# radiocosmology/cora

Measured on AMD Instinct MI355X. Metric: sky-maps/sec (nside=1024, lmax=2048, 256 freq), higher is better.
Workload: dtype f64

## Files before the change

### cora_amd/csrc/clarray.hip

```cpp
#include "common.h"

#include <cstring>
#include <type_traits>

#define CL_MAXZ 17

#define CL_XS 512
#define CL_LPT 9

__global__ void cl_transpose_kernel(const double *__restrict__ dd, const double *__restrict__ dv,
                                    const double *__restrict__ vv, int nkperp, int nkpar, double *__restrict__ tt) {
    __shared__ double tile[32][33];
    const double *src = blockIdx.z == 0 ? dd : (blockIdx.z == 1 ? dv : vv);
    double *dst = tt + (size_t)blockIdx.z * nkpar * CL_XS;
    const int x0 = blockIdx.y * 32, y0 = blockIdx.x * 32;
    const int tx = threadIdx.x & 31, ty = threadIdx.x >> 5;
    for (int r = ty; r < 32; r += 8) {
        const int x = x0 + r, y = y0 + tx;
        tile[r][tx] = (x < nkperp && y < nkpar) ? src[(size_t)x * nkpar + y] : 0.0;
    }
    __syncthreads();
    for (int r = ty; r < 32; r += 8) {
        const int y = y0 + r, x = x0 + tx;
        if (y < nkpar && x < CL_XS) dst[(size_t)y * CL_XS + x] = (x < nkperp) ? tile[tx][r] : 0.0;
    }
}

template <int ZINT>
__global__ void __launch_bounds__(256)
clarray21_kernel(const double *__restrict__ tt, int nkperp, int nkpar, double kperpmin, double xscale, double yscale,
                 const double *__restrict__ chi, const double *__restrict__ pfd, const double *__restrict__ fz,
                 const double *__restrict__ bz, int F, int zint_rt, const double *__restrict__ w,
                 const double *__restrict__ log10l, int nl, int l_base, const int2 *__restrict__ pairs,
                 double *__restrict__ scratch, int nl_total, int l_block) {
    const int zint = ZINT > 0 ? ZINT : zint_rt;
    extern __shared__ __attribute__((aligned(16))) double sm[];
    double *prof = sm;
    double *lxcs_s = sm + zint * (CL_XS + 2);
    double *par = lxcs_s + zint;
    int *ipar = reinterpret_cast<int *>(par + zint * zint * 8);
    const int PS = CL_XS + 2;
    const int tid = threadIdx.x;
    const int i = pairs[blockIdx.x].x, j = pairs[blockIdx.x].y;
    if (i < 0) return;
    const double ux = (double)nkperp - 1e-5, uy = (double)nkpar - 1e-5;
    const size_t tsz = (size_t)nkpar * CL_XS;

    double lxs[CL_LPT], acc[CL_LPT];
#pragma unroll
    for (int k = 0; k < CL_LPT; k++) {
        const int li = l_base + tid + 256 * k;
        lxs[k] = log10l[min(li, nl_total - 1)] * xscale;
        acc[k] = 0.0;
    }
    const int l_end = min(nl_total, l_base + 256 * CL_LPT);
    const double lx_lo = log10l[l_base] * xscale, lx_hi = log10l[l_end - 1] * xscale;
    const int kmax = (l_end - l_base + 255) / 256;

    int noclamp = 1;
    for (int t = tid; t < zint * zint; t += 256) {
        const int a = t / zint, b = t - a * zint;
        const int za = i * zint + a, zb = j * zint + b;
        const double x1 = chi[za], x2 = chi[zb];
        const double xc = 0.5 * (x1 + x2);
        const double lxc = log10(xc * kperpmin) * xscale;
        double yy = fabs(x2 - x1) * yscale;
        yy = yy < 0.0 ? 0.0 : (yy > uy ? uy : yy);
        int y0 = (int)yy;
        double wy = yy - (double)y0;
        if (y0 + 1 > nkpar - 1) {
            y0 = nkpar - 2;
            wy = 1.0;
        }
        const double W = w[a] * w[b] * pfd[za] * pfd[zb] / (xc * xc * M_PI);
        const double cdd = W * bz[za] * bz[zb];
        const double cdv = W * (fz[za] * bz[zb] + fz[zb] * bz[za]);
        const double cvv = W * fz[za] * fz[zb];
        double *pp = par + t * 8;
        pp[0] = cdd * (1.0 - wy);
        pp[1] = cdd * wy;
        pp[2] = cdv * (1.0 - wy);
        pp[3] = cdv * wy;
        pp[4] = cvv * (1.0 - wy);
        pp[5] = cvv * wy;
        pp[6] = lxc;
        double xhi = lx_hi - lxc, xlo = lx_lo - lxc;
        xhi = xhi < 0.0 ? 0.0 : (xhi > ux ? ux : xhi);
        xlo = xlo < 0.0 ? 0.0 : (xlo > ux ? ux : xlo);
        ipar[t * 4 + 0] = y0;
        ipar[t * 4 + 1] = (int)xlo;
        ipar[t * 4 + 2] = min((int)xhi + 2, nkperp);
        const double x2nd = (l_base + 1 < l_end ? log10l[l_base + 1] * xscale : lx_hi) - lxc;
        if (!(x2nd >= 0.0 && lx_hi - lxc <= ux)) noclamp = 0;
    }
    const bool all_fast = __syncthreads_and(noclamp) != 0;
    __shared__ int s_nsp;
    __shared__ double s_lxk[32];
    if (tid < 32) s_lxk[tid] = log10l[min(l_base + tid, nl_total - 1)] * xscale;
    if (tid < 64) {
        bool wide = false;
        if (l_base + tid + 1 < l_end) wide = (log10l[l_base + tid + 1] - log10l[l_base + tid]) * xscale >= 2.0;
        const unsigned long long m = __ballot(wide);
        if (tid == 0) s_nsp = m == ~0ull ? 32 : min(32, (int)__builtin_ctzll(~m));
    }

    for (int a = 0; a < zint; a++) {
        __syncthreads();
        if (ZINT > 0 && all_fast) {
            constexpr int ZN = ZINT > 0 ? ZINT : 1;
            const int nsp = min(s_nsp, l_end - l_base);
            const double lxd = log10l[min(l_base + nsp, nl_total - 1)] * xscale;
            int xlo = nkperp, xhi = 0;
#pragma unroll
            for (int b = 0; b < ZN; b++) {
                const double xx = fmin(fmax(lxd - par[(a * ZN + b) * 8 + 6], 0.0), ux);
                xlo = min(xlo, (int)xx);
                xhi = max(xhi, ipar[(a * ZN + b) * 4 + 2]);
            }
            if (nsp >= l_end - l_base) xlo = xhi;
            auto combine = [&](int b, const double (&v)[6]) {
                const double *pp = par + (a * ZN + b) * 8;
                return pp[0] * v[0] + pp[1] * v[1] + pp[2] * v[2] + pp[3] * v[3] + pp[4] * v[4] + pp[5] * v[5];
            };
            {
                constexpr int ZH = (ZN + 1) / 2;
                const int hb = tid >> 7, b0 = hb ? ZH : 0, nb = hb ? ZN - ZH : ZH;
                constexpr int QB = 3;
                for (int x = (xlo & ~1) + 2 * (tid & 127); x < xhi; x += 256) {
#pragma unroll
                    for (int q0 = 0; q0 < ZH; q0 += QB) {
                        double2 v[QB][6];
#pragma unroll
                        for (int q = 0; q < QB; q++) {
                            if (q0 + q < nb) {
                                const double *r0 = tt + (size_t)ipar[(a * ZN + b0 + q0 + q) * 4 + 0] * CL_XS + x, *r1 = r0 + CL_XS;
                                v[q][0] = *reinterpret_cast<const double2 *>(r0);
                                v[q][1] = *reinterpret_cast<const double2 *>(r1);
                                v[q][2] = *reinterpret_cast<const double2 *>(r0 + tsz);
                                v[q][3] = *reinterpret_cast<const double2 *>(r1 + tsz);
                                v[q][4] = *reinterpret_cast<const double2 *>(r0 + 2 * tsz);
                                v[q][5] = *reinterpret_cast<const double2 *>(r1 + 2 * tsz);
                            }
                        }
#pragma unroll
                        for (int q = 0; q < QB; q++) {
                            if (q0 + q < nb) {
                                const double *pp = par + (a * ZN + b0 + q0 + q) * 8;
                                double2 o;
                                o.x = pp[0] * v[q][0].x + pp[1] * v[q][1].x + pp[2] * v[q][2].x + pp[3] * v[q][3].x + pp[4] * v[q][4].x + pp[5] * v[q][5].x;
                                o.y = pp[0] * v[q][0].y + pp[1] * v[q][1].y + pp[2] * v[q][2].y + pp[3] * v[q][3].y + pp[4] * v[q][4].y + pp[5] * v[q][5].y;
                                *reinterpret_cast<double2 *>(prof + (b0 + q0 + q) * PS + x) = o;
                            }
// ... 20 lines not shown
            if (xhi == nkperp) {
                __syncthreads();
                if (tid < ZN) prof[tid * PS + nkperp] = prof[tid * PS + nkperp - 1];
            }
        } else
        for (int b = 0; b < zint; b++) {
            const int t = a * zint + b;
            const double *pp = par + t * 8;
            const double c0 = pp[0], c1 = pp[1], c2 = pp[2], c3 = pp[3], c4 = pp[4], c5 = pp[5];
            const int y0 = ipar[t * 4 + 0], x0r = ipar[t * 4 + 1], nx = ipar[t * 4 + 2];
            const double *r0 = tt + (size_t)y0 * CL_XS, *r1 = r0 + CL_XS;
            double *pb = prof + b * PS;
            for (int x = x0r + tid; x < nx; x += 256)
                pb[x] = c0 * r0[x] + c1 * r1[x] + c2 * r0[tsz + x] + c3 * r1[tsz + x] + c4 * r0[2 * tsz + x] +
                        c5 * r1[2 * tsz + x];
            if (tid == 0) lxcs_s[b] = pp[6];
            if (nx == nkperp && tid == ((nkperp - 1 - x0r) & 255)) pb[nkperp] = pb[nkperp - 1];
        }
        __syncthreads();
        double lxc_r[ZINT > 0 ? ZINT : 1];
        if constexpr (ZINT > 0) {
#pragma unroll
            for (int b = 0; b < ZINT; b++) lxc_r[b] = lxcs_s[b];
        }
        auto interp = [&](int b, double lx, double lxc, bool clamp) {
            double xx = lx - lxc;
            if (clamp) xx = fmin(fmax(xx, 0.0), ux);
            const int x0 = (int)xx;
            const double wx = __builtin_amdgcn_fract(xx);
            const double *pr = prof + b * PS + x0;
            const double s0 = pr[0], s1 = pr[1];
            return fma(wx, s1 - s0, s0);
        };
        auto interp_all = [&](auto fast_c) {
            constexpr bool FAST = decltype(fast_c)::value;
#pragma unroll
            for (int k = 0; k < CL_LPT; k++) {
                if (k < kmax && (k < kmax - 1 || l_base + tid + 256 * k < nl_total)) {
                    const bool clamp = !FAST || (k == 0 && tid == 0);
                    double s = 0.0;
                    if constexpr (ZINT > 0) {
#pragma unroll
                        for (int b = 0; b < ZINT; b++) s += interp(b, lxs[k], lxc_r[b], clamp);
                    } else {
                        for (int b = 0; b < zint; b++) s += interp(b, lxs[k], lxcs_s[b], clamp);
                    }
                    acc[k] += s;
                }
            }
        };
        if (all_fast) interp_all(std::true_type{});
        else interp_all(std::false_type{});
    }
#pragma unroll
    for (int k = 0; k < CL_LPT; k++) {
        const int li = l_base + tid + 256 * k;
        if (li < nl_total)
            scratch[((size_t)(li / l_block) * gridDim.x + blockIdx.x) * l_block + li % l_block] = acc[k];
    }
}

#define CL_BAND 32
__host__ __device__ static inline long cl_band_count(int n) {
    return n >= CL_BAND ? (long)CL_BAND * (n - (CL_BAND - 1)) + (long)(CL_BAND - 1) * CL_BAND / 2 : (long)n * (n + 1) / 2;
}
__host__ __device__ static inline int2 pair_of_index(long p, int F) {
    int B = 0;
    for (;; B++) {
        const long c = cl_band_count(F - CL_BAND * B);
        if (p < c) break;
        p -= c;
    }
    const int n = F - CL_BAND * B;
    const int nfull = n >= CL_BAND ? n - (CL_BAND - 1) : 0;
    int i, dd;
    if (p < (long)nfull * CL_BAND) {
        const int xq = (int)(p & 7), sq = (int)(p >> 3);
        i = sq >> 2;
        dd = 4 * xq + (sq & 3);
    } else {
        p -= (long)nfull * CL_BAND;
        int e = n >= CL_BAND ? CL_BAND - 1 : n;
        i = nfull;
        while (p >= e) {
            p -= e;
            e--;
// ... 127 lines not shown
                           const double *log10l, int nl, int pair_first, int pair_step, long npl_pad, int l_block,
                           double *out_pairs) {
    const size_t tt_bytes = sizeof(double) * 3 * (size_t)nkpar * CL_XS;
    double *tt = nullptr;
    int2 *dpairs = nullptr;
    int rc;
    if ((rc = corahip_ctx_scratch(ctx, 0, tt_bytes, (void **)&tt))) return rc;
    if ((rc = corahip_ctx_scratch(ctx, 2, sizeof(int2) * npl_pad, (void **)&dpairs))) return rc;
    const long key[4] = {F, pair_first, pair_step, npl_pad};
    if (ctx->pairs_ptr != (void *)dpairs || memcmp(key, ctx->pairs_key, sizeof(key)) != 0) {
        std::vector<int2> pairs((size_t)npl_pad, make_int2(-1, -1));
        long p = 0, k = 0;
        const long npairs_all = (long)F * (F + 1) / 2;
        for (; p < npairs_all; p++)
            if (p >= pair_first && (p - pair_first) % pair_step == 0) pairs[(size_t)k++] = pair_of_index(p, F);
        HIP_TRY(hipMemcpyAsync(dpairs, pairs.data(), sizeof(int2) * npl_pad, hipMemcpyHostToDevice, ctx->stream));
        HIP_TRY(hipStreamSynchronize(ctx->stream));
        memcpy(ctx->pairs_key, key, sizeof(key));
        ctx->pairs_ptr = (void *)dpairs;
    }
    const bool pinned = ctx->tt_pinned && ctx->tt_pin[0] == dd && ctx->tt_pin[1] == dv && ctx->tt_pin[2] == vv;
    if (!(pinned && ctx->tt_valid && ctx->tt_stream == ctx->stream && ctx->scratch_bytes[0] == tt_bytes)) {
        dim3 grid((nkpar + 31) / 32, CL_XS / 32, 3);
        cl_transpose_kernel<<<grid, 256, 0, ctx->stream>>>(dd, dv, vv, nkperp, nkpar, tt);
        LAUNCH_CHECK();
        ctx->tt_valid = pinned;
        ctx->tt_stream = ctx->stream;
    }
    const double xscale = (double)(nkperp - 1) / log10(kperpmax / kperpmin);
    const double yscale = kparmax / M_PI;
    const size_t shm = sizeof(double) * ((size_t)zint * (CL_XS + 2) + zint + (size_t)zint * zint * 10);
    auto kern = zint == 9 ? clarray21_kernel<9> : (zint == 5 ? clarray21_kernel<5> : (zint == 3 ? clarray21_kernel<3> : clarray21_kernel<0>));
    HIP_TRY(hipFuncSetAttribute((const void *)kern, hipFuncAttributeMaxDynamicSharedMemorySize, (int)shm));
    for (int l_base = 0; l_base < nl; l_base += 256 * CL_LPT) {
        kern<<<(unsigned)npl_pad, 256, shm, ctx->stream>>>(tt, nkperp, nkpar, kperpmin, xscale, yscale, chi, pfd, f, b, F, zint, w,
                                                          log10l, nl, l_base, dpairs, out_pairs, nl, l_block);
        LAUNCH_CHECK();
    }
    return 0;
}

int corahip_clarray_tables_pin(corahip_ctx *ctx, const double *dd, const double *dv, const double *vv, uint64_t generation) {
    ARG_CHECK(ctx != nullptr);
    if (dd == nullptr && generation != 0 && !(ctx->tt_pinned && ctx->tt_pin_gen == generation))
        return 0;
    const bool same = ctx->tt_pinned && dd && ctx->tt_pin[0] == dd && ctx->tt_pin[1] == dv && ctx->tt_pin[2] == vv &&
                      ctx->tt_pin_gen == generation;
    if (same) return 0;
    ctx->tt_pin[0] = dd;
    ctx->tt_pin[1] = dv;
    ctx->tt_pin[2] = vv;
    ctx->tt_pin_gen = generation;
    ctx->tt_pinned = dd != nullptr;
    ctx->tt_valid = false;
    return 0;
}

int corahip_clarray_table21cm(corahip_ctx *ctx, const double *dd, const double *dv, const double *vv, int nkperp,
                              int nkpar, double kperpmin, double kperpmax, double kparmax, const double *chi,
                              const double *pfd, const double *f, const double *b, int F, int zint, const double *w,
                              const double *log10l, int nl, double *out) {
    ARG_CHECK(ctx != nullptr && dd && dv && vv && chi && pfd && f && b && w && log10l && out);
    ARG_CHECK(nkperp >= 2 && nkperp < CL_XS && nkpar >= 2 && F >= 1 && zint >= 1 && zint <= CL_MAXZ && nl >= 1);
    ARG_CHECK(kperpmin > 0 && kperpmax > kperpmin && kparmax > 0);
    StageTimer t(ctx, "clarray");
    const long npairs = (long)F * (F + 1) / 2;
    double *scratch = nullptr;
    int rc;
    if ((rc = corahip_ctx_scratch(ctx, 1, sizeof(double) * (size_t)npairs * nl, (void **)&scratch))) return rc;
// ... 73 lines not shown
```

### cora_amd/csrc/common.h

```cpp
#pragma once
#include <hip/hip_runtime.h>

#include <cstdarg>
#include <cstdint>
#include <cstdio>
#include <map>
#include <string>
#include <type_traits>
#include <vector>

#include "../../include/corahip.h"
#include "dev_buf.h"

void corahip_set_error(const char *fmt, ...);

struct corahip_prof_entry {
    double total_ms = 0.0;
    int launches = 0;
};

struct corahip_pending_event {
    std::string name;
    hipEvent_t e0, e1;
};

struct corahip_linefft_plan {
    int n = 0, P = 0, logP = 0, blu = 0;
    int Pct = 0;
    dev_buf<double2> filt_ct;
    dev_buf<double2> tw;
    dev_buf<double2> chirp;
    dev_buf<double2> filt;
    dev_buf<double2> rtw;
};

#define CORAHIP_NSCRATCH 13
struct corahip_ctx {
    int device = 0;
    hipStream_t stream = nullptr;
    hipStream_t stream2 = nullptr;
    hipEvent_t ev_fork = nullptr, ev_join = nullptr;
    dev_buf<int> k5_tickets;
    dev_buf<unsigned> draw_slot_tab;
    int draw_slot_lmax = -1;
    bool mt_plist_ready = false;
    hipStream_t gen_stream = nullptr;
    hipEvent_t ev_ring[8] = {};
    const void *draw_pending = nullptr;
    hipEvent_t t0 = nullptr, t1 = nullptr;
    bool profile = false;
    std::map<std::string, corahip_prof_entry> prof;
    std::vector<corahip_pending_event> pending;
    int num_cu = 256;
    size_t total_mem = 0;
    dev_buf<char> scratch[CORAHIP_NSCRATCH];
    size_t scratch_bytes[CORAHIP_NSCRATCH] = {};
    int debug_poison = -1;
    const void *tt_pin[3] = {nullptr, nullptr, nullptr};
    uint64_t tt_pin_gen = 0;
    bool tt_pinned = false, tt_valid = false;
    hipStream_t tt_stream = nullptr;
    long pairs_key[4] = {-1, -1, -1, -1};
    void *pairs_ptr = nullptr;
    std::map<int, corahip_linefft_plan> linefft;
};

int corahip_ctx_scratch(corahip_ctx *ctx, int slot, size_t bytes, void **out);
int corahip_debug_fill(corahip_ctx *ctx, void *p, size_t bytes);

struct StageTimer {
    corahip_ctx *ctx;
    hipEvent_t e0 = nullptr, e1 = nullptr;
    const char *name;
    hipStream_t stream;
    StageTimer(corahip_ctx *c, const char *n, hipStream_t on = nullptr, bool other = false) : ctx(c), name(n), stream(other ? on : c->stream) {
        if (ctx->profile) {
            (void)hipEventCreate(&e0);
// ... 113 lines not shown
```

### cora_amd/csrc/draw.hip

```cpp
#include "common.h"

#include <cstdlib>
#include <type_traits>

#include "rng_dev.h"
#include "stream_internal.h"

__device__ static inline double2 philox_normal_pair(uint64_t seed, int l, int F, int nup, int m,
                                                    const double2 *lg = RNG_LOG_TAB, const double2 *sc = RNG_SC_TAB) {
    const uint64_t ctr = ((uint64_t)((uint32_t)l * (uint32_t)F + (uint32_t)nup) << 32) | (uint32_t)m;
    return philox_boxmuller(ctr, seed, lg, sc);
}

__global__ void normals_kernel(uint64_t seed, int lmax, int F, double *__restrict__ g) {
    const int l = blockIdx.y;
    const int lp1 = l + 1;
    const long n = (long)F * lp1;
    double *gl = g + (size_t)F * l * lp1;
    for (long q = (long)blockIdx.x * blockDim.x + threadIdx.x; q < n; q += (long)gridDim.x * blockDim.x) {
        const int m = (int)(q % lp1);
        const int nup = (int)(q / lp1);
        const double2 v = philox_normal_pair(seed, l, F, nup, m);
        gl[q] = v.x;
        gl[n + q] = v.y;
// ... 68 lines not shown
            }
        }
    }

    const double sc = 0.70710678118654752440;
    const long base = alm_idx(l, 0, lmax);
#pragma unroll
    for (int t = 0; t < NCT; t++) {
        const int col = col0 + 16 * t + ri;
        if (col >= 4 * Gout) continue;
#pragma unroll
        for (int r = 0; r < 4; r++) {
            const int ro = row0 + wave * 16 + kq + 4 * r;
            if (ro < nrow) {
                const int c = ro >= lp1 ? 1 : 0;
                const int m = ro - c * lp1;
                const long idx = (long)m * (2 * lmax + 1 - m) / 2 + l;
                (void)base;
                alm[((size_t)idx * Gout + (col >> 2)) * 8 + c * 4 + (col & 3)] = acc[t][r] * sc;
            }
        }
    }
}

__device__ static inline void draw_glds16(const void *gsrc, unsigned lds_byte_addr) {
    unsigned keep;
    const unsigned dst = __builtin_amdgcn_readfirstlane(lds_byte_addr);
    asm volatile("s_mov_b32 %0, m0\n\ts_mov_b32 m0, %2\n\ts_nop 0\n\tglobal_load_lds_dwordx4 %1, off\n\ts_mov_b32 m0, %0"
                 : "=&s"(keep)
                 : "v"(gsrc), "s"(dst)
                 : "memory");
}

#ifndef DRAW_STAMPS
#define DRAW_STAMPS 0
#endif
#if DRAW_STAMPS
__device__ unsigned long long g_draw_stamps[8];
#define DSTAMP(k) { unsigned long long _t; asm volatile("s_memtime %0\n\ts_waitcnt lgkmcnt(0)" : "=s"(_t)::"memory"); d_acc[k] += _t - d_last; d_last = _t; }
#else
#define DSTAMP(k)
#endif

#define DRAW_WAVES 8
#define DRAW_MB (16 * DRAW_WAVES)
#define DRAW_NBUF 3

static inline long draw_slots(int l_lo, int l_hi) {
    long n = 0;
    for (int l = l_lo; l <= l_hi; l++) n += (l / DRAW_MB) + 1;
    return n;
}

template <int NCT, bool FROMG = false, int NB = DRAW_NBUF>
__global__ void __launch_bounds__(64 * DRAW_WAVES, 2)
draw_rng_kernel(const double *__restrict__ T, size_t t_ldl, int rows, const int32_t *__restrict__ info,
                const double *__restrict__ zeros, uint64_t seed, const double *__restrict__ gsrc, size_t g_off, int l_lo,
                int l_hi, int lmax, int F, int nu0, int nu1, int cw, int nnu, int Gout, int nslots, int ncg0, int ncg,
                double *__restrict__ alm, unsigned *__restrict__ queue, const unsigned *__restrict__ slot_tab) {
    constexpr int NC = 16 * NCT;
    constexpr int ROWD = DRAW_KC;
    constexpr int BUF = NC * ROWD;
    constexpr int QPW = (NC / 4 + DRAW_WAVES - 1) / DRAW_WAVES;
    static_assert(QPW * DRAW_WAVES == NC / 4 || NC / 4 < DRAW_WAVES, "every staging wave issues the same number of pieces");
    extern __shared__ __attribute__((aligned(16))) double lds[];
    static_assert(NB == 3, "the counted waits below assume three stages");
    __shared__ double2 lg_s[257], sc_s[256];
    __shared__ int s_next[2];

    const int tid = threadIdx.x, lane = tid & 63;
    const int wave = __builtin_amdgcn_readfirstlane(tid >> 6);
    const int ri = lane & 15, kq = lane >> 4;
    const int nitems = nslots * ncg;
    const unsigned lds_base = (unsigned)(size_t)(__attribute__((address_space(3))) double *)lds;
#if DRAW_STAMPS
    unsigned long long d_acc[8] = {0, 0, 0, 0, 0, 0, 0, 0}, d_last;
    { unsigned long long _t; asm volatile("s_memtime %0\n\ts_waitcnt lgkmcnt(0)" : "=s"(_t)::"memory"); d_last = _t; }
#endif

    struct item_t {
        int l, mb, base0, lbase, lend, kmax, nchunk, c_full;
        bool tri_tail;
        const double *Tl;
// ... 190 lines not shown
                return __hiloint2double(hi, lo);
            };
#pragma unroll
            for (int t = 0; t < NCT; t++) {
                const int col = cur_lbase + 16 * t + (ri & ~3);
                const bool col_ok = col < cur_lend4;
#pragma unroll
                for (int r = 0; r < 4; r++) {
                    const double re = acc0[t][r] * sc, im = acc1[t][r] * sc;
                    const double re_a = quad(re, std::integral_constant<int, 0x88>{});
                    const double im_a = quad(im, std::integral_constant<int, 0x88>{});
                    const double re_b = quad(re, std::integral_constant<int, 0xDD>{});
                    const double im_b = quad(im, std::integral_constant<int, 0xDD>{});
                    const int m = mw + kq + 4 * r;
                    if (col_ok && m < lp1) {
                        const long idx = (long)m * (2 * lmax + 1 - m) / 2 + l;
                        *reinterpret_cast<double2 *>(alm + ((size_t)idx * Gout + (col >> 2)) * 8 + 2 * q) =
                            upper ? make_double2(im_a, im_b) : make_double2(re_a, re_b);
                    }
                }
            }
        }
        DSTAMP(5);
        if (!have_next) break;
    }
#if DRAW_STAMPS
    if (lane == 0) {
        for (int k = 0; k < 7; k++) atomicAdd(&g_draw_stamps[k], d_acc[k]);
        atomicAdd(&g_draw_stamps[7], 1ull);
    }
#endif
}

struct draw_chan {
    int nu0, nu1, cw, nnu;
};
static int draw_slot_table(corahip_ctx *ctx, int lmax, const unsigned **tab) {
    if (ctx->draw_slot_tab && ctx->draw_slot_lmax == lmax) {
        *tab = ctx->draw_slot_tab;
        return 0;
    }
    std::vector<unsigned> h;
    h.reserve((size_t)draw_slots(0, lmax));
    for (int l = lmax; l >= 0; l--)
        for (int mb = 0; mb <= l / DRAW_MB; mb++) h.push_back(((unsigned)l << 8) | (unsigned)mb);
    (void)ctx->draw_slot_tab.reset();
    ctx->draw_slot_lmax = -1;
    dev_buf<unsigned> d;
    HIP_TRY(d.alloc(h.size()));
    HIP_TRY(hipMemcpy(d, h.data(), sizeof(unsigned) * h.size(), hipMemcpyHostToDevice));
    ctx->draw_slot_tab = std::move(d);
    ctx->draw_slot_lmax = lmax;
    *tab = ctx->draw_slot_tab;
    return 0;
}

template <int NCT, bool FROMG = false, int NB = DRAW_NBUF>
static int launch_draw_rng(corahip_ctx *ctx, hipStream_t stream, const double *T, size_t t_ldl, int rows, const int32_t *info,
                           uint64_t seed, const double *gsrc, size_t g_off, int l_lo, int l_hi, int lmax, int F,
                           draw_chan ch, int Gout, double *alm) {
    constexpr int NC = 16 * NCT;
    const size_t shm = sizeof(double) * NB * NC * DRAW_KC;
    HIP_TRY(hipFuncSetAttribute((const void *)draw_rng_kernel<NCT, FROMG, NB>, hipFuncAttributeMaxDynamicSharedMemorySize,
                                (int)shm));
    char *zq = nullptr;
    int rc = corahip_ctx_scratch(ctx, 3, 8192, (void **)&zq);
    if (rc) return rc;
    HIP_TRY(hipMemsetAsync(zq, 0, 8192, stream));
    const int n0 = std::min(ch.cw, ch.nnu), n1 = ch.nnu - n0;
    const int ncg0 = (((n0 + 3) & ~3) + NC - 1) / NC, ncg = ncg0 + (((n1 + 3) & ~3) + NC - 1) / NC;
    const long nslots = draw_slots(l_lo, l_hi);
    const long nitems = nslots * ncg;
    ARG_CHECK(nitems < (1L << 30) && lmax < (1 << 24) && lmax / DRAW_MB < 256);
    const unsigned *slot_tab = nullptr;
    if ((rc = draw_slot_table(ctx, lmax, &slot_tab))) return rc;
    slot_tab += l_hi < lmax ? draw_slots(l_hi + 1, lmax) : 0;
    const int per_cu = (shm + 8300 > 80 * 1024) ? 1 : 2;
    dim3 grid((unsigned)std::min<long>(nitems, (long)ctx->num_cu * per_cu));
    draw_rng_kernel<NCT, FROMG, NB><<<grid, 64 * DRAW_WAVES, shm, stream>>>(T, t_ldl, rows, info, (const double *)zq, seed, gsrc,
                                                                        g_off, l_lo, l_hi, lmax, F, ch.nu0, ch.nu1, ch.cw,
                                                                        ch.nnu, Gout, (int)nslots, ncg0, ncg, alm,
                                                                        (unsigned *)(zq + 4096), slot_tab);
    LAUNCH_CHECK();
#if DRAW_STAMPS
    {
        unsigned long long hs[8], z[8] = {0};
        HIP_TRY(hipStreamSynchronize(stream));
        HIP_TRY(hipMemcpyFromSymbol(hs, HIP_SYMBOL(g_draw_stamps), sizeof(hs)));
        const double per = 1.0 / (double)std::max<unsigned long long>(hs[7], 1);
        fprintf(stderr, "K3 NCT=%d waves=%llu: cycles/wave  prologue %.0f wait+barrier %.0f (first chunk of an item %.0f) stage-issue %.0f rng+mfma %.0f next-item %.0f epilogue %.0f\n",
                NCT, hs[7], hs[0] * per, hs[1] * per, hs[6] * per, hs[2] * per, hs[3] * per, hs[4] * per, hs[5] * per);
        HIP_TRY(hipMemcpyToSymbol(HIP_SYMBOL(g_draw_stamps), z, sizeof(z)));
    }
#endif
    return 0;
}

__global__ void dev_to_square_kernel(const double *__restrict__ alm, int lmax, int nnu, int G,
                                     double *__restrict__ sq) {
    const int L = lmax + 1;
    const long n = (long)nnu * L * L;
    for (long q = (long)blockIdx.x * blockDim.x + threadIdx.x; q < n; q += (long)gridDim.x * blockDim.x) {
        const int m = (int)(q % L);
        const int l = (int)((q / L) % L);
        const int nu = (int)(q / ((long)L * L));
        double2 v = make_double2(0.0, 0.0);
        if (m <= l) {
            const long idx = (long)m * (2 * lmax + 1 - m) / 2 + l;
            const double *cell = alm + ((size_t)idx * G + (nu >> 2)) * 8 + (nu & 3);
            v = make_double2(cell[0], cell[4]);
        }
        *reinterpret_cast<double2 *>(sq + 2 * q) = v;
    }
}

// ... 53 lines not shown
        if (ncol <= 16) return launch_draw_rng<1, true>(ctx, stream, T, t_ldl, rows, info, 0, g, g_off, l_lo, l_hi, lmax, F, ch, Gout, alm_dev);
        if (ncol <= 32) return launch_draw_rng<2, true>(ctx, stream, T, t_ldl, rows, info, 0, g, g_off, l_lo, l_hi, lmax, F, ch, Gout, alm_dev);
        if (ncol <= 64) return launch_draw_rng<4, true>(ctx, stream, T, t_ldl, rows, info, 0, g, g_off, l_lo, l_hi, lmax, F, ch, Gout, alm_dev);
        return launch_draw_rng<8, true>(ctx, stream, T, t_ldl, rows, info, 0, g, g_off, l_lo, l_hi, lmax, F, ch, Gout, alm_dev);
    }
    ARG_CHECK(!chan_folded(ch));
    const int ncol = 4 * Gout, nu0 = ch.nu0, nnu = ch.nnu, t_row0 = rows ? nu0 : 0;
    if (ncol <= 16) return launch_draw<1>(ctx, stream, T, t_ldl, t_row0, info, g, g_off, l_lo, l_hi, lmax, F, nu0, nnu, Gout, alm_dev);
    if (ncol <= 32) return launch_draw<2>(ctx, stream, T, t_ldl, t_row0, info, g, g_off, l_lo, l_hi, lmax, F, nu0, nnu, Gout, alm_dev);
    if (ncol <= 64) return launch_draw<4>(ctx, stream, T, t_ldl, t_row0, info, g, g_off, l_lo, l_hi, lmax, F, nu0, nnu, Gout, alm_dev);
    if (ncol <= 128) return launch_draw<8>(ctx, stream, T, t_ldl, t_row0, info, g, g_off, l_lo, l_hi, lmax, F, nu0, nnu, Gout, alm_dev);
    return launch_draw<16>(ctx, stream, T, t_ldl, t_row0, info, g, g_off, l_lo, l_hi, lmax, F, nu0, nnu, Gout, alm_dev);
}

static int draw_host_stream(corahip_ctx *ctx, const double *T, int rows, const int32_t *info, const double *g, int lmax, int F,
                            draw_chan ch, double *alm_dev) {
    StageTimer t(ctx, "draw");
    return draw_stream_range(ctx, ctx->stream, T, rows, info, g, 0, 0, lmax, lmax, F, ch, alm_dev);
}

static int draw_philox(corahip_ctx *ctx, const double *T, int rows, const int32_t *info, uint64_t seed, int lmax, int F,
                       draw_chan ch, double *alm_dev) {
    if (F & 1) {
        double *g = nullptr;
        int rc = corahip_ctx_scratch(ctx, 1, sizeof(double) * 2 * (size_t)F * nalm_of(lmax), (void **)&g);
        if (rc) return rc;
        if ((rc = corahip_normals_philox(ctx, seed, lmax, F, g))) return rc;
        return draw_host_stream(ctx, T, rows, info, g, lmax, F, ch, alm_dev);
    }
    StageTimer t(ctx, "draw");
    const int Gout = (ch.nnu + 3) / 4;
    const size_t t_ldl = rows ? (size_t)ch.nnu * F : (size_t)F * F;
    const int ncol = chan_ncol(ch);
    if (ncol <= 16) return launch_draw_rng<1>(ctx, ctx->stream, T, t_ldl, rows, info, seed, nullptr, 0, 0, lmax, lmax, F, ch, Gout, alm_dev);
    if (ncol <= 32) return launch_draw_rng<2>(ctx, ctx->stream, T, t_ldl, rows, info, seed, nullptr, 0, 0, lmax, lmax, F, ch, Gout, alm_dev);
    if (ncol <= 64) return launch_draw_rng<4>(ctx, ctx->stream, T, t_ldl, rows, info, seed, nullptr, 0, 0, lmax, lmax, F, ch, Gout, alm_dev);
    return launch_draw_rng<8>(ctx, ctx->stream, T, t_ldl, rows, info, seed, nullptr, 0, 0, lmax, lmax, F, ch, Gout, alm_dev);
}

static int chan_of(const corahip_chanset *set, int F, draw_chan &ch) {
    ARG_CHECK(set != nullptr && (set->nchunks == 1 || set->nchunks == 2) && set->chunk_nnu >= 1);
    ARG_CHECK(set->nu0[0] >= 0 && set->nu0[0] + set->chunk_nnu <= F);
    if (set->nchunks == 2) {
        ARG_CHECK(set->chunk_nnu % 4 == 0);
        ARG_CHECK(set->nu0[1] >= set->nu0[0] + set->chunk_nnu && set->nu0[1] + set->chunk_nnu <= F);
        ch = draw_chan{set->nu0[0], set->nu0[1], set->chunk_nnu, 2 * set->chunk_nnu};
    } else {
        ch = draw_chan{set->nu0[0], 0, set->chunk_nnu, set->chunk_nnu};
    }
    return 0;
}

int corahip_draw_alm_philox(corahip_ctx *ctx, const double *T, const int32_t *info, uint64_t seed, int lmax, int F,
                            int nu0, int nnu, double *alm_dev) {
    ARG_CHECK(ctx != nullptr && T != nullptr && alm_dev != nullptr);
    ARG_CHECK(lmax >= 0 && F >= 1 && nu0 >= 0 && nnu >= 1 && nu0 + nnu <= F);
    return draw_philox(ctx, T, 0, info, seed, lmax, F, draw_chan{nu0, 0, nnu, nnu}, alm_dev);
}

int corahip_draw_alm_philox_rows(corahip_ctx *ctx, const double *T_rows, const int32_t *info, uint64_t seed, int lmax,
                                 int F, int nu0, int nnu, double *alm_dev) {
    ARG_CHECK(ctx != nullptr && T_rows != nullptr && alm_dev != nullptr);
    ARG_CHECK(lmax >= 0 && F >= 1 && nu0 >= 0 && nnu >= 1 && nu0 + nnu <= F);
    return draw_philox(ctx, T_rows, 1, info, seed, lmax, F, draw_chan{nu0, 0, nnu, nnu}, alm_dev);
}

// ... 54 lines not shown
```

Measured before the change: 3298.

## Replace per-l sub-sample interpolation with knot-based row sums in clarray kernel

When all sub-sample centre offsets lie within half a cell of a central offset, the kernel accumulates per-column row sums S and first-moment sums E over the z sub-samples. Each l is then evaluated with one linear interpolation of S corrected by E, instead of interpolating every sub-sample separately. Multipoles whose bracketing cell is ambiguous are put on a dirty list and still go through the exact per-sample path. The change also adds a launch-bounds occupancy hint and extra shared memory, and is on by default with an environment variable to disable it.

```diff
diff --git a/cora_amd/csrc/clarray.hip b/cora_amd/csrc/clarray.hip
--- a/cora_amd/csrc/clarray.hip
+++ b/cora_amd/csrc/clarray.hip
@@ -7,6 +7,9 @@
 
 #define CL_XS 512
 #define CL_LPT 9
+#define CL_KN_CAP 512
+#define CL_KN_MARGIN 0x1p-20
+#define CL_KN_DMAX (0.5 - 0x1p-20)
 
 __global__ void cl_transpose_kernel(const double *__restrict__ dd, const double *__restrict__ dv,
                                     const double *__restrict__ vv, int nkperp, int nkpar, double *__restrict__ tt) {
@@ -26,13 +29,18 @@
     }
 }
 
+__device__ static inline double cl_mul_rn(double a, double b) {
+#pragma clang fp contract(off)
+    return a * b;
+}
+
 template <int ZINT>
-__global__ void __launch_bounds__(256)
+__global__ void __launch_bounds__(256, 3)
 clarray21_kernel(const double *__restrict__ tt, int nkperp, int nkpar, double kperpmin, double xscale, double yscale,
                  const double *__restrict__ chi, const double *__restrict__ pfd, const double *__restrict__ fz,
                  const double *__restrict__ bz, int F, int zint_rt, const double *__restrict__ w,
                  const double *__restrict__ log10l, int nl, int l_base, const int2 *__restrict__ pairs,
-                 double *__restrict__ scratch, int nl_total, int l_block) {
+                 double *__restrict__ scratch, int nl_total, int l_block, int knots_on) {
     const int zint = ZINT > 0 ? ZINT : zint_rt;
     extern __shared__ __attribute__((aligned(16))) double sm[];
     double *prof = sm;
@@ -96,7 +104,7 @@
     const bool all_fast = __syncthreads_and(noclamp) != 0;
     __shared__ int s_nsp;
     __shared__ double s_lxk[32];
-    if (tid < 32) s_lxk[tid] = log10l[min(l_base + tid, nl_total - 1)] * xscale;
+    if (tid < 32) s_lxk[tid] = cl_mul_rn(log10l[min(l_base + tid, nl_total - 1)], xscale);
     if (tid < 64) {
         bool wide = false;
         if (l_base + tid + 1 < l_end) wide = (log10l[l_base + tid + 1] - log10l[l_base + tid]) * xscale >= 2.0;
@@ -104,7 +112,86 @@
         if (tid == 0) s_nsp = m == ~0ull ? 32 : min(32, (int)__builtin_ctzll(~m));
     }
 
-    for (int a = 0; a < zint; a++) {
+    constexpr int ZQ = ZINT > 0 ? ZINT : 1;
+    __shared__ double s_dlim[2];
+    __shared__ int s_kok, s_ndirty;
+    __shared__ unsigned short s_dlist[CL_KN_CAP];
+    __shared__ double s_dlx[CL_KN_CAP];
+    __shared__ double s_early[32][4];
+    bool knots = false, kn_early = false, kn_eclean = false;
+    unsigned kn_dirty = 0;
+    double cstar = 0.0;
+    double kn_S[2] = {0.0, 0.0}, kn_E[2] = {0.0, 0.0};
+    double kn_lacc[CL_KN_CAP / 256];
+    int kn_lidx[CL_KN_CAP / 256];
+    int kn_xlo = 0, kn_xhi = 0;
+    if constexpr (ZINT > 0) {
+        if (knots_on && all_fast) {
+            if (tid < 64) {
+                const double c0 = par[((ZQ / 2) * ZQ + ZQ / 2) * 8 + 6];
+                double lo = 0.0, hi = 0.0;
+                int ok = 1;
+                for (int t = tid; t < ZQ * ZQ; t += 64) {
+                    const double d = par[t * 8 + 6] - c0;
+                    par[t * 8 + 7] = d;
+                    lo = fmin(lo, d);
+                    hi = fmax(hi, d);
+                    if (ipar[t * 4 + 2] == nkperp) ok = 0;
+                }
+#pragma unroll
+                for (int s = 32; s >= 1; s >>= 1) {
+                    lo = fmin(lo, __shfl_xor(lo, s));
+                    hi = fmax(hi, __shfl_xor(hi, s));
+                    ok &= __shfl_xor(ok, s);
+                }
+                if (tid == 0) {
+                    s_dlim[0] = lo;
+                    s_dlim[1] = hi;
+                    s_kok = ok && fmax(-lo, hi) < CL_KN_DMAX;
+                    s_ndirty = 0;
+                }
+            }
+            __syncthreads();
+            knots = s_kok != 0;
+        }
+        if (knots) {
+            cstar = par[((ZQ / 2) * ZQ + ZQ / 2) * 8 + 6];
+            const double dmin = s_dlim[0], dmax = s_dlim[1];
+            const int nsp = min(s_nsp, l_end - l_base);
+            kn_early = tid < nsp;
+            if (tid < 32) s_early[tid][0] = s_early[tid][1] = s_early[tid][2] = s_early[tid][3] = 0.0;
+#pragma unroll
+            for (int k = 0; k < CL_LPT; k++) {
+                const int e = tid + 256 * k;
+                if (l_base + e >= nl_total) continue;
+                const double lxe = cl_mul_rn(log10l[l_base + e], xscale);
+                const double xs = lxe - cstar;
+                const double lo = xs - dmax - CL_KN_MARGIN, hi = xs - dmin + CL_KN_MARGIN;
+                const bool clean = lo >= 0.0 && (int)lo == (int)hi;
+                if (k == 0 && kn_early) {
+                    kn_eclean = clean;
+                } else if (!clean) {
+                    kn_dirty |= 1u << k;
+                    const int slot = atomicAdd(&s_ndirty, 1);
+                    if (slot < CL_KN_CAP) {
+                        s_dlist[slot] = (unsigned short)e;
+                        s_dlx[slot] = lxe;
+                    }
+                }
+            }
+            __syncthreads();
+            const int nd = s_ndirty;
+            if (nd > CL_KN_CAP) knots = false;
+#pragma unroll
+            for (int q = 0; q < CL_KN_CAP / 256; q++) {
+                kn_lidx[q] = (knots && tid + 256 * q < nd) ? (int)s_dlist[tid + 256 * q] : -1;
+                kn_lacc[q] = 0.0;
+            }
+        }
+    }
+
+    auto round = [&](int a, auto kn_c) {
+        constexpr bool KN = decltype(kn_c)::value;
         __syncthreads();
         if (ZINT > 0 && all_fast) {
             constexpr int ZN = ZINT > 0 ? ZINT : 1;
@@ -118,6 +205,8 @@
                 xhi = max(xhi, ipar[(a * ZN + b) * 4 + 2]);
             }
             if (nsp >= l_end - l_base) xlo = xhi;
+            kn_xlo = xlo & ~1;
+            kn_xhi = xhi;
             auto combine = [&](int b, const double (&v)[6]) {
                 const double *pp = par + (a * ZN + b) * 8;
                 return pp[0] * v[0] + pp[1] * v[1] + pp[2] * v[2] + pp[3] * v[3] + pp[4] * v[4] + pp[5] * v[5];
@@ -204,6 +293,46 @@
             const double s0 = pr[0], s1 = pr[1];
             return fma(wx, s1 - s0, s0);
         };
+        if constexpr (ZINT > 0 && KN) {
+            const double *dl_r = par + a * ZQ * 8 + 7;
+            auto rowsum = [&](int x, double &S, double &E) {
+                const double *pr = prof + x;
+                double t = pr[0], e = dl_r[0] * t;
+#pragma unroll
+                for (int b = 1; b < ZQ; b++) {
+                    const double s = pr[b * PS];
+                    t += s;
+                    e = fma(dl_r[8 * b], s, e);
+                }
+                S += t;
+                E += e;
+            };
+            auto sub_sum = [&](double lx) {
+                double s = 0.0;
+#pragma unroll
+                for (int b = 0; b < ZQ; b++) s += interp(b, lx, lxc_r[b], true);
+                return s;
+            };
+#pragma unroll
+            for (int r = 0; r < 2; r++) {
+                const int x = tid + 256 * r;
+                if (x >= kn_xlo && x < kn_xhi) rowsum(x, kn_S[r], kn_E[r]);
+            }
+            if (kn_early) {
+                double *se = s_early[tid];
+                if (kn_eclean) {
+                    const int x = (int)(s_lxk[tid] - cstar);
+                    rowsum(x, se[0], se[2]);
+                    rowsum(x + 1, se[1], se[3]);
+                } else {
+                    se[0] += sub_sum(s_lxk[tid]);
+                }
+            }
+#pragma unroll
+            for (int q = 0; q < CL_KN_CAP / 256; q++)
+                if (kn_lidx[q] >= 0) kn_lacc[q] += sub_sum(s_dlx[tid + 256 * q]);
+            return;
+        }
         auto interp_all = [&](auto fast_c) {
             constexpr bool FAST = decltype(fast_c)::value;
 #pragma unroll
@@ -223,7 +352,47 @@
         };
         if (all_fast) interp_all(std::true_type{});
         else interp_all(std::false_type{});
-    }
+    };
+    auto slot_of = [&](int li) {
+        return ((size_t)(li / l_block) * gridDim.x + blockIdx.x) * l_block + li % l_block;
+    };
+    if constexpr (ZINT > 0) {
+        if (knots) {
+            for (int a = 0; a < ZINT; a++) round(a, std::true_type{});
+            __syncthreads();
+#pragma unroll
+            for (int r = 0; r < 2; r++) {
+                prof[tid + 256 * r] = kn_S[r];
+                prof[PS + tid + 256 * r] = kn_E[r];
+            }
+            __syncthreads();
+            auto knot_value = [](double xs, double S0, double S1, double E0, double E1) {
+                return fma(__builtin_amdgcn_fract(xs), S1 - S0, S0) - (E1 - E0);
+            };
+#pragma unroll
+            for (int k = 0; k < CL_LPT; k++) {
+                const int li = l_base + tid + 256 * k;
+                if (li >= nl_total) continue;
+                double v;
+                if (k == 0 && kn_early) {
+                    const double *se = s_early[tid];
+                    v = kn_eclean ? knot_value(s_lxk[tid] - cstar, se[0], se[1], se[2], se[3]) : se[0];
+                } else if ((kn_dirty >> k) & 1) {
+                    continue;
+                } else {
+                    const double xs = cl_mul_rn(log10l[li], xscale) - cstar;
+                    const double *pr = prof + (int)xs;
+                    v = knot_value(xs, pr[0], pr[1], pr[PS], pr[PS + 1]);
+                }
+                scratch[slot_of(li)] = v;
+            }
+#pragma unroll
+            for (int q = 0; q < CL_KN_CAP / 256; q++)
+                if (kn_lidx[q] >= 0) scratch[slot_of(l_base + kn_lidx[q])] = kn_lacc[q];
+            return;
+        }
+    }
+    for (int a = 0; a < zint; a++) round(a, std::false_type{});
 #pragma unroll
     for (int k = 0; k < CL_LPT; k++) {
         const int li = l_base + tid + 256 * k;
@@ -417,9 +586,11 @@
     const size_t shm = sizeof(double) * ((size_t)zint * (CL_XS + 2) + zint + (size_t)zint * zint * 10);
     auto kern = zint == 9 ? clarray21_kernel<9> : (zint == 5 ? clarray21_kernel<5> : (zint == 3 ? clarray21_kernel<3> : clarray21_kernel<0>));
     HIP_TRY(hipFuncSetAttribute((const void *)kern, hipFuncAttributeMaxDynamicSharedMemorySize, (int)shm));
+    const char *kn_env = getenv("CORAHIP_K1_KNOTS");
+    const int knots_on = !(kn_env && kn_env[0] == '0' && kn_env[1] == 0);
     for (int l_base = 0; l_base < nl; l_base += 256 * CL_LPT) {
         kern<<<(unsigned)npl_pad, 256, shm, ctx->stream>>>(tt, nkperp, nkpar, kperpmin, xscale, yscale, chi, pfd, f, b, F, zint, w,
-                                                          log10l, nl, l_base, dpairs, out_pairs, nl, l_block);
+                                                          log10l, nl, l_base, dpairs, out_pairs, nl, l_block, knots_on);
         LAUNCH_CHECK();
     }
     return 0;
```

Result: no change. 3325 (median of 6 runs) (+0.8%).

## Add wide 256-column draw kernel with half-height m blocks for large channel counts

Applied to the files above, without the earlier changes.

Adds a new draw kernel that covers 256 output columns per block, with 16 MFMA tiles per wave and only 8 m rows per wave. It uses double-buffered LDS staging fed by scalar-base global-to-LDS loads. For more than 128 channels, one block now handles all frequencies, so the Philox normals are generated once per (l,m) instead of once per column group. The slot table becomes per-m-block-size. The trade-off is higher accumulator register pressure, larger LDS use, and smaller m blocks that need more work items.

```diff
diff --git a/cora_amd/csrc/common.h b/cora_amd/csrc/common.h
--- a/cora_amd/csrc/common.h
+++ b/cora_amd/csrc/common.h
@@ -41,8 +41,8 @@
     hipStream_t stream2 = nullptr;
     hipEvent_t ev_fork = nullptr, ev_join = nullptr;
     dev_buf<int> k5_tickets;
-    dev_buf<unsigned> draw_slot_tab;
-    int draw_slot_lmax = -1;
+    dev_buf<unsigned> draw_slot_tab[2];
+    int draw_slot_lmax[2] = {-1, -1};
     bool mt_plist_ready = false;
     hipStream_t gen_stream = nullptr;
     hipEvent_t ev_ring[8] = {};
diff --git a/cora_amd/csrc/draw.hip b/cora_amd/csrc/draw.hip
--- a/cora_amd/csrc/draw.hip
+++ b/cora_amd/csrc/draw.hip
@@ -124,6 +124,15 @@
                  : "memory");
 }
 
+__device__ static inline void draw_glds16_s(const void *sbase, unsigned lane_byte_off, unsigned lds_byte_addr) {
+    unsigned keep;
+    const unsigned dst = __builtin_amdgcn_readfirstlane(lds_byte_addr);
+    asm volatile("s_mov_b32 %0, m0\n\ts_mov_b32 m0, %3\n\ts_nop 0\n\tglobal_load_lds_dwordx4 %1, %2\n\ts_mov_b32 m0, %0"
+                 : "=&s"(keep)
+                 : "v"(lane_byte_off), "s"(sbase), "s"(dst)
+                 : "memory");
+}
+
 #ifndef DRAW_STAMPS
 #define DRAW_STAMPS 0
 #endif
@@ -138,9 +147,15 @@
 #define DRAW_MB (16 * DRAW_WAVES)
 #define DRAW_NBUF 3
 
-static inline long draw_slots(int l_lo, int l_hi) {
+#define DRAW_WNCT 16
+#define DRAW_WMB (8 * DRAW_WAVES)
+#ifndef DRAW_WIDE
+#define DRAW_WIDE 1
+#endif
+
+static inline long draw_slots(int l_lo, int l_hi, int mb = DRAW_MB) {
     long n = 0;
-    for (int l = l_lo; l <= l_hi; l++) n += (l / DRAW_MB) + 1;
+    for (int l = l_lo; l <= l_hi; l++) n += (l / mb) + 1;
     return n;
 }
 
@@ -397,55 +412,263 @@
 #endif
 }
 
+__global__ void __launch_bounds__(64 * DRAW_WAVES, 2)
+draw_wide_kernel(const double *__restrict__ T, size_t t_ldl, int rows, const int32_t *__restrict__ info,
+                 const double *__restrict__ zeros, uint64_t seed, int lmax, int F, int nu0, int nu1, int cw, int nnu, int Gout,
+                 int nslots, int ncg0, int ncg, double *__restrict__ alm, unsigned *__restrict__ queue,
+                 const unsigned *__restrict__ slot_tab) {
+    constexpr int NCT = DRAW_WNCT, NC = 16 * NCT;
+    constexpr int ROWD = DRAW_KC;
+    constexpr int BUF = NC * ROWD;
+    constexpr int QPW = NC / 4 / DRAW_WAVES;
+    extern __shared__ __attribute__((aligned(16))) double lds[];
+    __shared__ double2 lg_s[257], sc_s[256];
+    __shared__ int s_next[2];
+
+    const int tid = threadIdx.x, lane = tid & 63;
+    const int wave = __builtin_amdgcn_readfirstlane(tid >> 6);
+    const int ri = lane & 15, kq = lane >> 4;
+    const bool odd = ri & 1;
+    const int nitems = nslots * ncg;
+    const unsigned lds_base = (unsigned)(size_t)(__attribute__((address_space(3))) double *)lds;
+#if DRAW_STAMPS
+    unsigned long long d_acc[8] = {0, 0, 0, 0, 0, 0, 0, 0}, d_last;
+    { unsigned long long _t; asm volatile("s_memtime %0\n\ts_waitcnt lgkmcnt(0)" : "=s"(_t)::"memory"); d_last = _t; }
+#endif
+
+    struct item_t {
+        int l, mb, base0, lbase, lend, kmax, nchunk, c_full;
+        bool tri_tail;
+        const double *Tl;
+    };
+    auto decode = [&](int it) {
+        item_t w;
+        const int cg = ncg - 1 - it / nslots;
+        const int s = it - (it / nslots) * nslots;
+        const unsigned e = slot_tab[s];
+        const int l = (int)(e >> 8), mb = (int)(e & 255u);
+        w.l = l;
+        w.mb = mb;
+        const bool second = cg >= ncg0;
+        w.lbase = second ? cw + (cg - ncg0) * NC : cg * NC;
+        w.lend = second ? nnu : min(cw, nnu);
+        w.base0 = second ? nu1 + (cg - ncg0) * NC : nu0 + cg * NC;
+        const bool dense = (info == nullptr) || (info[l] != 0);
+        w.kmax = dense ? F : min(F, w.base0 + NC);
+        w.nchunk = (w.kmax + DRAW_KC - 1) / DRAW_KC;
+        w.tri_tail = !dense && (w.base0 % DRAW_KC) == 0;
+        w.c_full = w.tri_tail ? min(w.nchunk, w.base0 / DRAW_KC) : w.nchunk;
+        w.Tl = T + (size_t)l * t_ldl + (size_t)(rows ? w.lbase : w.base0) * F;
+        return w;
+    };
+    const int n_lane = 4 * wave + (lane >> 4), slot_lane = (lane & 15) ^ (n_lane & 15);
+    const unsigned src_lane_off = (unsigned)(((size_t)n_lane * F + 2 * slot_lane) * sizeof(double));
+    auto stage = [&](const item_t &w, int c, int slot, auto first_c) {
+        constexpr int FIRST = decltype(first_c)::value;
+        const int k0 = c * DRAW_KC;
+        const int n_valid = min(w.lend - w.lbase, F - w.base0);
+        const unsigned dst = lds_base + (unsigned)((slot * BUF + 4 * wave * ROWD) * sizeof(double));
+        constexpr unsigned DST_STEP = 4 * DRAW_WAVES * ROWD * sizeof(double);
+        if (n_valid >= NC && k0 + DRAW_KC <= F) {
+            const double *src = w.Tl + k0;
+#pragma unroll
+            for (int it = FIRST; it < QPW; it++) draw_glds16_s(src + (size_t)(4 * DRAW_WAVES * it) * F, src_lane_off, dst + it * DST_STEP);
+        } else {
+#pragma unroll
+            for (int it = FIRST; it < QPW; it++) {
+                const int n = n_lane + 4 * DRAW_WAVES * it;
+                const int k = k0 + 2 * slot_lane;
+                const double *src = zeros;
+                if (n < n_valid && k + 1 < F) src = w.Tl + (size_t)n * F + k;
+                draw_glds16(src, dst + it * DST_STEP);
+            }
+        }
+    };
+    constexpr std::integral_constant<int, 0> whole_stage{};
+
+    for (int i = tid; i < 257; i += 64 * DRAW_WAVES) lg_s[i] = RNG_LOG_TAB[i];
+    for (int i = tid; i < 256; i += 64 * DRAW_WAVES) sc_s[i] = RNG_SC_TAB[i];
+
+    int item = blockIdx.x;
+    if (item >= nitems) return;
+    item_t w = decode(item);
+    int ring = 0, par = 0;
+    stage(w, 0, 0, whole_stage);
+    DSTAMP(0);
+
+    for (;;) {
+        if (tid == 0) s_next[par] = (int)(gridDim.x + atomicAdd(queue, 1u));
+        const int l = w.l, lp1 = w.l + 1;
+        const int mw = w.mb * DRAW_WMB + 8 * wave;
+        const bool wave_has_rows = mw < lp1;
+        const int m_lane = mw + (ri >> 1);
+        const int kmax = w.kmax, nchunk = w.nchunk;
+        d4_t acc[NCT];
+#pragma unroll
+        for (int t = 0; t < NCT; t++) acc[t] = (d4_t){0.0, 0.0, 0.0, 0.0};
+        auto half_steps = [&](auto tmin_c, const double *sb, int k0, auto half_c) {
+            constexpr int TMIN = decltype(tmin_c)::value;
+            constexpr int half = decltype(half_c)::value;
+#pragma unroll
+            for (int j = 2 * half; j < 2 * half + 2; j++) {
+                const double2 g = philox_normal_pair(seed, l, F, k0 + 8 * j + (odd ? 4 : 0) + kq, m_lane, lg_s, sc_s);
+                const double give = odd ? g.x : g.y;
+                int lo = __double2loint(give), hi = __double2hiint(give);
+                lo = __builtin_amdgcn_update_dpp(lo, lo, 0xB1, 0xF, 0xF, false);
+                hi = __builtin_amdgcn_update_dpp(hi, hi, 0xB1, 0xF, 0xF, false);
+                const double got = __hiloint2double(hi, lo);
+                const double a[2] = {odd ? got : g.x, odd ? g.y : got};
+#pragma unroll
+                for (int s = 0; s < 2; s++) {
+                    const int kl = 8 * j + 4 * s + kq;
+                    const double *brow = sb + ri * ROWD + 2 * ((kl >> 1) ^ ri) + (kl & 1);
+#pragma unroll
+                    for (int t0 = 0; t0 < NCT; t0 += 8) {
+                        double bv[8];
+#pragma unroll
+                        for (int t = t0; t < t0 + 8; t++)
+                            if (t >= TMIN) bv[t - t0] = brow[16 * t * ROWD];
+#pragma unroll
+                        for (int t = t0; t < t0 + 8; t++)
+                            if (t >= TMIN) acc[t] = __builtin_amdgcn_mfma_f64_16x16x4f64(a[s], bv[t - t0], acc[t], 0, 0, 0);
+                    }
+                }
+            }
+        };
+        auto chunk_begin = [&](int c, auto next_first) {
+            asm volatile("s_waitcnt vmcnt(0)" ::: "memory");
+            __syncthreads();
+#if DRAW_STAMPS
+            if (c == 0) { DSTAMP(6); } else
+#endif
+            DSTAMP(1);
+            if (c + 1 < nchunk) stage(w, c + 1, (ring + c + 1) & 1, next_first);
+            DSTAMP(2);
+        };
+        int c = 0;
+        for (; c < w.c_full; c++) {
+            chunk_begin(c, whole_stage);
+            if (!wave_has_rows) continue;
+            const double *sb = lds + ((ring + c) & 1) * BUF;
+            half_steps(std::integral_constant<int, 0>{}, sb, c * DRAW_KC, std::integral_constant<int, 0>{});
+            if (c * DRAW_KC + 16 < kmax) half_steps(std::integral_constant<int, 0>{}, sb, c * DRAW_KC, std::integral_constant<int, 1>{});
+            DSTAMP(3);
+        }
+        static_for<NC / DRAW_KC>([&](auto jc) {
+            constexpr int J = decltype(jc)::value;
+            if (c >= nchunk) return;
+            chunk_begin(c, std::integral_constant<int, (J + 1 < QPW ? J + 1 : QPW)>{});
+            if (wave_has_rows) {
+                const double *sb = lds + ((ring + c) & 1) * BUF;
+                half_steps(std::integral_constant<int, 2 * J>{}, sb, c * DRAW_KC, std::integral_constant<int, 0>{});
+                if (c * DRAW_KC + 16 < kmax)
+                    half_steps(std::integral_constant<int, 2 * J + 1>{}, sb, c * DRAW_KC, std::integral_constant<int, 1>{});
+                DSTAMP(3);
+            }
+            c++;
+        });
+
+        ring = (ring + nchunk) & 1;
+        const int cur_lbase = w.lbase, cur_lend4 = (w.lend + 3) & ~3;
+        item = __builtin_amdgcn_readfirstlane(s_next[par]);
+        par ^= 1;
+        const bool have_next = item < nitems;
+        if (have_next) {
+            w = decode(item);
+            stage(w, 0, ring, whole_stage);
+        }
+        DSTAMP(4);
+
+        if (wave_has_rows) {
+            const double sc = 0.70710678118654752440;
+            double *cell[4];
+            bool m_ok[4];
+#pragma unroll
+            for (int r = 0; r < 4; r++) {
+                const int m = mw + (kq >> 1) + 2 * r;
+                const long idx = (long)m * (2 * lmax + 1 - m) / 2 + l;
+                m_ok[r] = m < lp1;
+                cell[r] = alm + ((size_t)idx * Gout + ((cur_lbase + (ri & ~3)) >> 2)) * 8 + 4 * (kq & 1) + (ri & 3);
+            }
+            const int ncol_lane = cur_lend4 - cur_lbase - (ri & ~3);
+#pragma unroll
+            for (int t = 0; t < NCT; t++) {
+                const bool col_ok = 16 * t < ncol_lane;
+#pragma unroll
+                for (int r = 0; r < 4; r++)
+                    if (col_ok && m_ok[r]) cell[r][32 * t] = acc[t][r] * sc;
+            }
+        }
+        DSTAMP(5);
+        if (!have_next) break;
+    }
+#if DRAW_STAMPS
+    if (lane == 0) {
+        for (int k = 0; k < 7; k++) atomicAdd(&g_draw_stamps[k], d_acc[k]);
+        atomicAdd(&g_draw_stamps[7], 1ull);
+    }
+#endif
+}
+
 struct draw_chan {
     int nu0, nu1, cw, nnu;
 };
-static int draw_slot_table(corahip_ctx *ctx, int lmax, const unsigned **tab) {
-    if (ctx->draw_slot_tab && ctx->draw_slot_lmax == lmax) {
-        *tab = ctx->draw_slot_tab;
+static int draw_slot_table(corahip_ctx *ctx, int lmax, int mb, const unsigned **tab) {
+    const int which = mb == DRAW_MB ? 0 : 1;
+    if (ctx->draw_slot_tab[which] && ctx->draw_slot_lmax[which] == lmax) {
+        *tab = ctx->draw_slot_tab[which];
         return 0;
     }
     std::vector<unsigned> h;
-    h.reserve((size_t)draw_slots(0, lmax));
+    h.reserve((size_t)draw_slots(0, lmax, mb));
     for (int l = lmax; l >= 0; l--)
-        for (int mb = 0; mb <= l / DRAW_MB; mb++) h.push_back(((unsigned)l << 8) | (unsigned)mb);
-    (void)ctx->draw_slot_tab.reset();
-    ctx->draw_slot_lmax = -1;
+        for (int b = 0; b <= l / mb; b++) h.push_back(((unsigned)l << 8) | (unsigned)b);
+    (void)ctx->draw_slot_tab[which].reset();
+    ctx->draw_slot_lmax[which] = -1;
     dev_buf<unsigned> d;
     HIP_TRY(d.alloc(h.size()));
     HIP_TRY(hipMemcpy(d, h.data(), sizeof(unsigned) * h.size(), hipMemcpyHostToDevice));
-    ctx->draw_slot_tab = std::move(d);
-    ctx->draw_slot_lmax = lmax;
-    *tab = ctx->draw_slot_tab;
+    ctx->draw_slot_tab[which] = std::move(d);
+    ctx->draw_slot_lmax[which] = lmax;
+    *tab = ctx->draw_slot_tab[which];
     return 0;
 }
 
-template <int NCT, bool FROMG = false, int NB = DRAW_NBUF>
+template <int NCT, bool FROMG = false>
 static int launch_draw_rng(corahip_ctx *ctx, hipStream_t stream, const double *T, size_t t_ldl, int rows, const int32_t *info,
                            uint64_t seed, const double *gsrc, size_t g_off, int l_lo, int l_hi, int lmax, int F,
                            draw_chan ch, int Gout, double *alm) {
-    constexpr int NC = 16 * NCT;
+    constexpr bool WIDE = NCT == DRAW_WNCT;
+    static_assert(!(WIDE && FROMG), "the wide shape generates its normals");
+    constexpr int NC = 16 * NCT, MB = WIDE ? DRAW_WMB : DRAW_MB, NB = WIDE ? 2 : DRAW_NBUF;
     const size_t shm = sizeof(double) * NB * NC * DRAW_KC;
-    HIP_TRY(hipFuncSetAttribute((const void *)draw_rng_kernel<NCT, FROMG, NB>, hipFuncAttributeMaxDynamicSharedMemorySize,
-                                (int)shm));
+    const void *kernel;
+    if constexpr (WIDE) kernel = (const void *)draw_wide_kernel;
+    else kernel = (const void *)draw_rng_kernel<NCT, FROMG, NB>;
+    HIP_TRY(hipFuncSetAttribute(kernel, hipFuncAttributeMaxDynamicSharedMemorySize, (int)shm));
     char *zq = nullptr;
     int rc = corahip_ctx_scratch(ctx, 3, 8192, (void **)&zq);
     if (rc) return rc;
     HIP_TRY(hipMemsetAsync(zq, 0, 8192, stream));
     const int n0 = std::min(ch.cw, ch.nnu), n1 = ch.nnu - n0;
     const int ncg0 = (((n0 + 3) & ~3) + NC - 1) / NC, ncg = ncg0 + (((n1 + 3) & ~3) + NC - 1) / NC;
-    const long nslots = draw_slots(l_lo, l_hi);
+    const long nslots = draw_slots(l_lo, l_hi, MB);
     const long nitems = nslots * ncg;
-    ARG_CHECK(nitems < (1L << 30) && lmax < (1 << 24) && lmax / DRAW_MB < 256);
+    ARG_CHECK(nitems < (1L << 30) && lmax < (1 << 24) && lmax / MB < 256);
     const unsigned *slot_tab = nullptr;
-    if ((rc = draw_slot_table(ctx, lmax, &slot_tab))) return rc;
-    slot_tab += l_hi < lmax ? draw_slots(l_hi + 1, lmax) : 0;
+    if ((rc = draw_slot_table(ctx, lmax, MB, &slot_tab))) return rc;
+    slot_tab += l_hi < lmax ? draw_slots(l_hi + 1, lmax, MB) : 0;
     const int per_cu = (shm + 8300 > 80 * 1024) ? 1 : 2;
     dim3 grid((unsigned)std::min<long>(nitems, (long)ctx->num_cu * per_cu));
-    draw_rng_kernel<NCT, FROMG, NB><<<grid, 64 * DRAW_WAVES, shm, stream>>>(T, t_ldl, rows, info, (const double *)zq, seed, gsrc,
-                                                                        g_off, l_lo, l_hi, lmax, F, ch.nu0, ch.nu1, ch.cw,
-                                                                        ch.nnu, Gout, (int)nslots, ncg0, ncg, alm,
-                                                                        (unsigned *)(zq + 4096), slot_tab);
+    if constexpr (WIDE)
+        draw_wide_kernel<<<grid, 64 * DRAW_WAVES, shm, stream>>>(T, t_ldl, rows, info, (const double *)zq, seed, lmax, F, ch.nu0,
+                                                                ch.nu1, ch.cw, ch.nnu, Gout, (int)nslots, ncg0, ncg, alm,
+                                                                (unsigned *)(zq + 4096), slot_tab);
+    else
+        draw_rng_kernel<NCT, FROMG, NB><<<grid, 64 * DRAW_WAVES, shm, stream>>>(T, t_ldl, rows, info, (const double *)zq, seed, gsrc,
+                                                                            g_off, l_lo, l_hi, lmax, F, ch.nu0, ch.nu1, ch.cw,
+                                                                            ch.nnu, Gout, (int)nslots, ncg0, ncg, alm,
+                                                                            (unsigned *)(zq + 4096), slot_tab);
     LAUNCH_CHECK();
 #if DRAW_STAMPS
     {
@@ -565,6 +788,9 @@
     const int Gout = (ch.nnu + 3) / 4;
     const size_t t_ldl = rows ? (size_t)ch.nnu * F : (size_t)F * F;
     const int ncol = chan_ncol(ch);
+#if DRAW_WIDE
+    if (ncol > 128) return launch_draw_rng<DRAW_WNCT>(ctx, ctx->stream, T, t_ldl, rows, info, seed, nullptr, 0, 0, lmax, lmax, F, ch, Gout, alm_dev);
+#endif
     if (ncol <= 16) return launch_draw_rng<1>(ctx, ctx->stream, T, t_ldl, rows, info, seed, nullptr, 0, 0, lmax, lmax, F, ch, Gout, alm_dev);
     if (ncol <= 32) return launch_draw_rng<2>(ctx, ctx->stream, T, t_ldl, rows, info, seed, nullptr, 0, 0, lmax, lmax, F, ch, Gout, alm_dev);
     if (ncol <= 64) return launch_draw_rng<4>(ctx, ctx->stream, T, t_ldl, rows, info, seed, nullptr, 0, 0, lmax, lmax, F, ch, Gout, alm_dev);
```

Measured after the change: 3293 before, 3336 after, median of 6. 1.01x the previous value.
